# JiaxuanYou/graph-pooling

Hardware: AMD Instinct MI355X
Metric: graphs/sec fwd+bwd, DD padded batch N_max=500 (higher is better)
Workload: dtype f32; 1 GPU; S-DD: DD-shaped padded batch, B=20/GPU, N_max=500, F=89, H=E=20, K=50, L=3, 1 pool; graphs_per_gpu=20, global_batch=20, linkpred=False, hip_graph=True, parallelism=dp1

## Files before the change

### graph_pooling_amd/_lib.py

```python
from __future__ import annotations

import ctypes as C
import os
import threading

_HERE = os.path.dirname(os.path.abspath(__file__))
LIB_PATH = os.environ.get("DP_LIB") or os.path.join(_HERE, "libdiffpool_hip.so")

DP_MAX_LAYERS = 8
DP_MAX_LEVELS = 4
DP_MAX_PRED = 4

F_ADD_SELF, F_NORMALIZE, F_RELU, F_BN, F_LAST_ONLY = 1, 2, 4, 8, 16
MODE_EVAL, MODE_TRAIN = 0, 1
ERR_DEVICE = -4
DEVERR_BARRIER, DEVERR_NONFINITE_GRAD = 1, 2
SAVE_S, SAVE_XPOOL, SAVE_ADJPOOL, SAVE_Z, SAVE_ZASSIGN, SAVE_ARGMAX = 0, 1, 2, 3, 4, 5


class StackCfg(C.Structure):
    _fields_ = [("n_layers", C.c_int),
                ("dims", C.c_int * (DP_MAX_LAYERS + 1)),
                ("w_off", C.c_long * DP_MAX_LAYERS),
                ("b_off", C.c_long * DP_MAX_LAYERS),
# ... 9 lines not shown
                ("assign_pred_w_off", C.c_long * DP_MAX_LEVELS),
                ("assign_pred_b_off", C.c_long * DP_MAX_LEVELS),
                ("n_pred", C.c_int),
                ("pred_dims", C.c_int * (DP_MAX_PRED + 2)),
                ("pred_w_off", C.c_long * (DP_MAX_PRED + 1)),
                ("pred_b_off", C.c_long * (DP_MAX_PRED + 1)),
                ("flags", C.c_int),
                ("readout", C.c_int),
                ("s2s_off", C.c_long * 6),
                ("mask_readout", C.c_int),
                ("n_params", C.c_long),
                ("n_graph_params", C.c_long),
                ("bn_world", C.c_int),
                ("exchange", C.c_void_p),
                ("exchange_user", C.c_void_p)]


EXCHANGE_FN = C.CFUNCTYPE(C.c_int, C.c_void_p, C.c_void_p, C.c_void_p, C.c_size_t, C.c_void_p)


_P = C.c_void_p
_I = C.c_int
_L = C.c_long
_F = C.c_float
_Z = C.c_size_t

_PROTOS = {
    "dp_version": (_I, []),
    "dp_last_error_string": (C.c_char_p, []),
    "dp_device_error": (_I, [_I]),
    "dp_device_error_describe": (C.c_char_p, [_I]),
    "dp_profile_level0": (_I, [_I]),
    "dp_profile_level0_read": (_I, [_I, C.POINTER(C.c_double), C.POINTER(_I)]),
    "dp_sizeof_encoder_cfg": (_Z, []),
    "dp_bgemm_f32": (_I, [_P, _P, _P, _P, _I, _I, _I, _I, _I, _I, _I, _L, _L, _L, _I, _I, _F, _F, _I, _P]),
    "dp_bgemm_split_bf16": (_I, [_P, _P, _P, _I, _I, _I, _I, _I, _I, _I, _L, _L, _L, _I, _I, _F, _P]),
    "dp_adj_aggregate": (_I, [_P, _P, _I, _P, _I, _I, _I, _I, _I, _F, _P]),
    "dp_adj_pack_ld": (_I, [_I]),
    "dp_adj_pack_bytes": (_Z, [_I, _I]),
    "dp_adj_pack": (_I, [_P, _P, _P, _P, _I, _I, _P]),
    "dp_adj_aggregate_packed_workspace_bytes": (_Z, [_I, _I, _I]),
    "dp_adj_aggregate_packed": (_I, [_P, _P, _P, _P, _P, _I, _P, _I, _I, _I, _I, _I, _F, _I, _P, _Z, _P]),
    "dp_gcn_layer_workspace_bytes": (_Z, [_I, _I, _I, _I]),
    "dp_gcn_layer_fwd": (_I, [_P, _I, _P, _P, _P, _P, _I, _P, _I, _I, _I, _I, _I, _P, _Z, _P]),
    "dp_gcn_layer_bwd": (_I, [_P, _I, _P, _P, _P, _I, _P, _P, _I, _P, _I, _P, _P, _P, _I, _I, _I, _I, _I, _P, _Z, _P]),
    "dp_bn_node_workspace_bytes": (_Z, [_I, _I, _I]),
    "dp_bn_node_fwd": (_I, [_P, _I, _P, _I, _P, _I, _I, _I, _I, _P, _Z, _P]),
    "dp_bn_node_bwd": (_I, [_P, _I, _P, _I, _P, _P, _I, _P, _I, _I, _I, _I, _I, _P, _Z, _P]),
    "dp_assign_workspace_bytes": (_Z, [_I, _I, _I, _I]),
    "dp_assign_softmax_mask_fwd": (_I, [_P, _I, _P, _P, _P, _P, _I, _I, _I, _I, _P, _Z, _P]),
    "dp_assign_softmax_mask_bwd": (_I, [_P, _I, _P, _P, _P, _P, _P, _I, _P, _P, _I, _I, _I, _I, _P, _Z, _P]),
    "dp_pool_fwd": (_I, [_P, _P, _I, _P, _P, _P, _P, _I, _I, _I, _I, _P]),
    "dp_pool_bwd_workspace_bytes": (_Z, [_I, _I, _I, _I]),
    "dp_pool_bwd": (_I, [_P, _P, _I, _P, _P, _P, _P, _P, _P, _I, _P, _I, _I, _I, _I, _P, _Z, _P]),
    "dp_masked_max_fwd": (_I, [_P, _I, _P, _P, _I, _P, _I, _I, _I, _P]),
    "dp_masked_max_bwd": (_I, [_P, _I, _P, _P, _I, _I, _I, _I, _P]),
    "dp_linkpred_workspace_bytes": (_Z, [_I, _I, _I]),
    "dp_linkpred_loss_fwd": (_I, [_P, _P, _P, _P, _I, _I, _I, _P, _Z, _P]),
    "dp_linkpred_loss_bwd": (_I, [_P, _P, _P, _P, _P, _I, _I, _I, _I, _P, _Z, _P]),
    "dp_cross_entropy_fwd": (_I, [_P, _P, _P, _P, _I, _I, _P]),
    "dp_cross_entropy_bwd": (_I, [_P, _P, _P, _P, _I, _I, _P]),
    "dp_set2set_save_bytes": (_Z, [_I, _I, _I]),
    "dp_set2set_plan": (_I, [_I, _I]),
    "dp_set2set_fwd": (_I, [_P, _I, _P, _P, _P, _P, _P, _P, _P, _I, _I, _I, _P, _Z, _P]),
    "dp_set2set_bwd_workspace_bytes": (_Z, [_I, _I, _I]),
    "dp_set2set_bwd": (_I, [_P, _I, _P, _P, _P, _P, _P, _P, _P, _P, _P, _I, _P, _P, _P, _P, _P, _P,
# ... 106 lines not shown
```

### graph_pooling_amd/csrc/dp_level0.hip

```cpp
#include "dp_common.h"
#include <utility>
#include <vector>

namespace dp {

#ifdef DP_STAMP
__device__ unsigned long long g_l0_stamps[3][64];
#define L0_STAMP(i)                                                                                    \
    do {                                                                                               \
        if (threadIdx.x == 0 && (wid == 0 || wid == (int)gridDim.x / 2 || wid == (int)gridDim.x - 1)) \
            g_l0_stamps[wid == 0 ? 0 : (wid == (int)gridDim.x - 1 ? 2 : 1)][i] = __builtin_amdgcn_s_memtime(); \
    } while (0)
#else
#define L0_STAMP(i) \
    do {            \
    } while (0)
#endif

namespace {

typedef float f32x4 __attribute__((ext_vector_type(4)));
typedef float f32x4_u __attribute__((ext_vector_type(4), aligned(4)));
typedef short s16x8 __attribute__((ext_vector_type(8)));
typedef __bf16 bf16x8 __attribute__((ext_vector_type(8)));
typedef unsigned short u16x4 __attribute__((ext_vector_type(4)));
typedef unsigned short u16x8 __attribute__((ext_vector_type(8)));

constexpr int L0_NT = 512;
constexpr int L0_NW = 8;
constexpr int L0_TEAMS = L0_NT / 16;
constexpr int L0_NK = 4;
constexpr int L0_BPAIRS = 4;
constexpr float L0_L2_EPS = 1e-12f;
constexpr float L0_BN_EPS = 1e-5f;
constexpr int L0_SPIN_LIMIT = 1 << 22;

constexpr int BAR_GCOUNT = 0, BAR_DONE = 32, BAR_GFLAG = 48, BAR_ERR = 64, BAR_SEQ = 96, BAR_GRAPH0 = 128;
constexpr int BAR_GSTRIDE = 48;

__device__ __forceinline__ int ag_ld(int* p) { return __hip_atomic_load(p, __ATOMIC_RELAXED, __HIP_MEMORY_SCOPE_AGENT); }
__device__ __forceinline__ void ag_st(int* p, int v) { __hip_atomic_store(p, v, __ATOMIC_RELAXED, __HIP_MEMORY_SCOPE_AGENT); }
__device__ __forceinline__ int ag_add(int* p, int v) { return __hip_atomic_fetch_add(p, v, __ATOMIC_RELAXED, __HIP_MEMORY_SCOPE_AGENT); }

struct L0Args {
    Level0Fwd f;
    int T, RB;
    int ldp;
    int K8;
    int steps;
    int epad;
    long vs_off[DP_MAX_LAYERS + 1];
    int lds_act[2];
    int lds_scr;
    int scr_floats;
    int* dev_err;
    int spin_limit, target_bias;
    long zero_n16;
};

template <bool TA, bool TB, typename Store>
__device__ inline void l0_mma(const float* A, int lda, const float* B, int ldb, int M, int N, int K, Store store,
                              int wave_shift = 0) {
    const int lane = threadIdx.x & 63;
    const int wave = ((threadIdx.x >> 6) + L0_NW - wave_shift % L0_NW) % L0_NW;
    const int l15 = lane & 15, kq = lane >> 4;
    const int tm = (M + 15) / 16, tn = (N + 15) / 16;
    const int sa4 = 4 * (TA ? lda : 1), sb4 = 4 * (TB ? 1 : ldb);
    for (int t = wave; t < tm * tn; t += L0_NW) {
        const int tr = t / tn, tc = t - tr * tn;
        const int i = tr * 16 + l15, j = tc * 16 + l15;
        const float* ap = (TA ? A + min(i, M - 1) : A + min(i, M - 1) * lda) + kq * (sa4 >> 2);
        const float* bp = (TB ? B + min(j, N - 1) * ldb : B + min(j, N - 1)) + kq * (sb4 >> 2);
        f32x4 acc0 = (f32x4){0.f, 0.f, 0.f, 0.f}, acc1 = acc0;
        int k = 0;
        float pa[4], pb[4], qa[4], qb[4];
        auto ld = [&](float (&xa)[4], float (&xb)[4]) {
            xa[0] = ap[0]; xa[1] = ap[sa4]; xa[2] = ap[2 * sa4]; xa[3] = ap[3 * sa4];
            xb[0] = bp[0]; xb[1] = bp[sb4]; xb[2] = bp[2 * sb4]; xb[3] = bp[3 * sb4];
            ap += 4 * sa4;
            bp += 4 * sb4;
        };
        auto mm = [&](const float (&xa)[4], const float (&xb)[4]) {
            acc0 = __builtin_amdgcn_mfma_f32_16x16x4f32(xa[0], xb[0], acc0, 0, 0, 0);
            acc1 = __builtin_amdgcn_mfma_f32_16x16x4f32(xa[1], xb[1], acc1, 0, 0, 0);
// ... 114 lines not shown
            q[u] = *reinterpret_cast<const f32x4_u*>(src + 4 * min(base + u * L0_NT + (int)threadIdx.x, nq - 1));
#pragma unroll
        for (int u = 0; u < QN; ++u) {
            const int e4 = base + u * L0_NT + (int)threadIdx.x;
            if (e4 < nq) *reinterpret_cast<f32x4*>(dst + 4 * e4) = q[u];
        }
    }
    if (te < count) dst[te] = tail;
    for (int e = count + (int)threadIdx.x; e < zero_to; e += L0_NT) dst[e] = 0.f;
}

__device__ inline void l0_write_split(ScBuf vsb, const float* PT, int ct, int CTt, int K8, int k8_0, int nk8, int nrows) {
    const long pl = (long)CTt * K8 * 128;
    const int items = nk8 * CTt * 16;
    for (int item = threadIdx.x; item < items; item += L0_NT) {
        const int c = item & 15, t = item >> 4;
        const int k8l = t / CTt, cb = t - k8l * CTt;
        const int vc = cb * 16 + c, lr = k8l * 8;
        u16x8 h, m, l;
#pragma unroll
        for (int j = 0; j < 8; ++j) {
            const float v = (vc < ct && lr + j < nrows) ? PT[(lr + j) * ct + min(vc, ct - 1)] : 0.f;
            unsigned short hh, mm, ll;
            bf16_split3(v, hh, mm, ll);
            h[j] = hh; m[j] = mm; l[j] = ll;
        }
        const long o = vs_index(0, CTt, K8, cb, k8_0 + k8l, c, 0);
        sc_st16(vsb, (unsigned)(o * 2), __builtin_bit_cast(u32x4, h));
        sc_st16(vsb, (unsigned)((o + pl) * 2), __builtin_bit_cast(u32x4, m));
        sc_st16(vsb, (unsigned)((o + 2 * pl) * 2), __builtin_bit_cast(u32x4, l));
    }
}

template <int MI, int CTH>
__device__ __forceinline__ void l0_agg_bf16(const unsigned short* Alds, int ldp, const unsigned short* vsp, int CTt, int K8,
                                            int steps, int rot, int cb0, f32x4 (&acc)[MI][CTH]) {
    int lane = threadIdx.x & 63;
    asm volatile("" : "+v"(lane));
    const int kh = __builtin_amdgcn_readfirstlane(threadIdx.x >> 6) & 3;
    const int l15 = lane & 15, kq = lane >> 4;
    auto eff = [&](int step) {
        const int s2 = min(step, steps - 1) + rot;
        return s2 >= steps ? s2 - steps : s2;
    };
    auto load_b = [&](int step, s16x8 (&dst)[3][CTH]) {
        const int st = eff(step);
#pragma unroll
        for (int p = 0; p < 3; ++p)
#pragma unroll
            for (int cbi = 0; cbi < CTH; ++cbi) {
                const int cb = min(cb0 + cbi, CTt - 1);
                const long o = ((((long)p * CTt + cb) * K8 + st * 4 + kq) * 16 + l15) * 8;
                dst[p][cbi] = *reinterpret_cast<const s16x8*>(vsp + o);
            }
    };
    auto mma = [&](int step, const s16x8 (&bf)[3][CTH]) {
        s16x8 av[MI];
#pragma unroll
        for (int rb = 0; rb < MI; ++rb)
            av[rb] = *reinterpret_cast<const s16x8*>(Alds + (rb * 16 + l15) * ldp + eff(step) * 32 + kq * 8);
#pragma unroll
        for (int p = 2; p >= 0; --p)
#pragma unroll
            for (int rb = 0; rb < MI; ++rb)
#pragma unroll
                for (int cbi = 0; cbi < CTH; ++cbi)
// ... 141 lines not shown
        const bool in = row < nrows && c8 * 8 < ld;
        const u32x4 v = in ? s.q[u] : (u32x4){0u, 0u, 0u, 0u};
        if (c8 * 8 + 8 <= ldp) *reinterpret_cast<u32x4*>(Alds + row * ldp + c8 * 8) = v;
    }
}

template <int MI>
__global__ __launch_bounds__(L0_NT) void k_level0_fwd(L0Args a) {
    constexpr int RB = MI * 16;
    extern __shared__ __attribute__((aligned(16))) float lds[];
    const Level0Fwd& f = a.f;
    const int tid = threadIdx.x, lane = tid & 63;
    const int tl = tid & 15, team = tid >> 4;
    const int N = f.N, G = f.G, L = f.L;
    int wid;
    {
        const int nwg = gridDim.x, xcd = blockIdx.x & 7, idx = blockIdx.x >> 3;
        const int qd = nwg >> 3, rm = nwg & 7;
        wid = (xcd < rm ? xcd * (qd + 1) : rm * (qd + 1) + (xcd - rm) * qd) + idx;
    }
    const int b = wid / a.T, rb = wid - b * a.T;
    const int r0 = rb * RB;
    const int nrows = min(RB, N - r0);
    const int nb = f.num_nodes ? min(f.num_nodes[b], N) : N;
    const int rot = (rb * 4) % a.steps;
    L0_STAMP(0);

    unsigned short* Alds = reinterpret_cast<unsigned short*>(lds);
    float* ACT0 = lds + a.lds_act[0];
    float* ACT1 = lds + a.lds_act[1];
    float* SCR = lds + a.lds_scr;
    float* BIAS = lds + a.lds_scr + a.scr_floats;
    int* sflag = reinterpret_cast<int*>(BIAS + (2 * DP_MAX_LAYERS + 1) * 64);
    if (tid < 4) sflag[tid] = 0;
    L0Epoch ep{0};
    const unsigned seq = (unsigned)f.bar[BAR_SEQ];

    auto vs_wr = [&](int pass, int CTt) {
        return sc_buf(f.vs + a.vs_off[pass] + (long)b * 3 * CTt * a.K8 * 128, (size_t)3 * CTt * a.K8 * 128 * 2);
    };
    auto vs_rd = [&](int pass, int CTt) { return f.vs + a.vs_off[pass] + (long)b * 3 * CTt * a.K8 * 128; };

    if (wid == 0) {
        if (f.next_bar && tid < 64) f.next_bar[tid] = 0;
        if (tid == 64) ag_st(f.bar + BAR_ERR, 0);
    }
    L0_STAMP(1);
    const int din0_0 = f.st[0].dims[0], din0_1 = G == 2 ? f.st[1].dims[0] : 0;
    bool bad = false;
    float* const X0s0 = SCR;
    float* const X0s1 = X0s0 + RB * din0_0;
    float* const W0s0 = X0s1 + RB * din0_1;
    float* const W0s1 = W0s0 + ((din0_0 * f.st[0].dims[1] + 3) & ~3);
    float* const PT = W0s1 + (G == 2 ? ((din0_1 * f.st[1].dims[1] + 3) & ~3) : 0);
    const auto side_loads = [&]() {
        l0_copy_in<4>(X0s0, f.x0[0] + ((long)b * N + r0) * din0_0, nrows * din0_0, RB * din0_0);
        l0_copy_in<4>(W0s0, f.params + f.st[0].w_off[0], din0_0 * f.st[0].dims[1]);
        if (G == 2) {
            l0_copy_in<4>(X0s1, f.x0[1] + ((long)b * N + r0) * din0_1, nrows * din0_1, RB * din0_1);
            l0_copy_in<4>(W0s1, f.params + f.st[1].w_off[0], din0_1 * f.st[1].dims[1]);
        }
        for (int e = tid; e < (2 * L + 1) * 64; e += L0_NT) {
            const int slot = e >> 6, c = e & 63;
            float v0 = 0.f;
            if (slot < 2 * L) {
                const int l = slot >> 1, g = slot & 1;
                if (g < G && f.st[g].b_off[l] >= 0 && c < f.st[g].dims[l + 1]) v0 = f.params[f.st[g].b_off[l] + c];
            } else if (G == 2 && f.bp_off >= 0 && c < f.K) {
                v0 = f.params[f.bp_off + c];
            }
            BIAS[(slot < 2 * L ? slot : 2 * DP_MAX_LAYERS) * 64 + c] = v0;
        }
    };
    if (f.A) {
// ... 33 lines not shown
        for (int seg = 1; seg < segs; ++seg) {
            l0_stage_issue<MI>(q, rows, f.pk_ld, nrows, seg);
            l0_stage_commit<MI>(q, Alds, a.ldp, f.pk_ld, nrows, seg);
        }
    }
    L0_STAMP(2);
    if (f.zero_p) {
        uint4* zp = reinterpret_cast<uint4*>(f.zero_p);
        const long nwg = gridDim.x, per = (a.zero_n16 + nwg - 1) / nwg;
        const long end = min(a.zero_n16, ((long)wid + 1) * per);
        for (long i = (long)wid * per + tid; i < end; i += L0_NT) zp[i] = make_uint4(0, 0, 0, 0);
    }
    if (__any(bad) && lane == 0) sflag[2] = 1;
    lds_barrier();
    L0_STAMP(3);
    const bool blk_bad = sflag[2] != 0;
    if (blk_bad && tid == 0) {
        ag_st(f.bar + BAR_GRAPH0 + b * BAR_GSTRIDE + 32, 1);
        ag_st(f.bar + BAR_GFLAG, 1);
    }
    if (f.A) {
        const ScBuf atb = sc_buf(f.pkAt + (long)b * N * f.pk_ld, (size_t)N * f.pk_ld * 2);
        constexpr int P8 = RB / 8;
        for (int e = tid; e < N * P8; e += L0_NT) {
            const int k = e / P8, i8 = e - k * P8;
            if (r0 + i8 * 8 < f.pk_ld) {
                u16x8 h;
#pragma unroll
                for (int j = 0; j < 8; ++j) h[j] = Alds[(i8 * 8 + j) * a.ldp + k];
                sc_st16(atb, (unsigned)(((long)k * f.pk_ld + r0 + i8 * 8) * 2), __builtin_bit_cast(u32x4, h));
            }
        }
    }
    L0_STAMP(4);
    int ct = f.st[0].dims[1] + (G == 2 ? f.st[1].dims[1] : 0);
    for (int g = 0; g < G; ++g) {
        const int dout = f.st[g].dims[1], c0 = g ? f.st[0].dims[1] : 0;
        l0_mma<false, false>(g ? X0s1 : X0s0, g ? din0_1 : din0_0, g ? W0s1 : W0s0, dout, RB, dout, g ? din0_1 : din0_0,
                             [&](int r, int c, float v) { PT[r * ct + c0 + c] = v; }, g * 3);
    }
    lds_barrier();
    L0_STAMP(5);
    const int k8_0 = r0 / 8;
    const int nk8 = min(rb == a.T - 1 ? a.K8 - k8_0 : RB / 8, a.K8 - k8_0);
    {
        const int CTt = (ct + 15) / 16;
        l0_write_split(vs_wr(0, CTt), PT, ct, CTt, a.K8, k8_0, nk8, nrows);
    }
    L0_STAMP(6);
    bool ok = l0_barrier(a, b, sflag, ep);
    L0_STAMP(7);
    const bool exact = !f.A || ag_ld(f.bar + BAR_GRAPH0 + b * BAR_GSTRIDE + 32) == 0;
    const float* Arows = f.A + ((long)b * N + r0) * N;
    const float* Acols = f.A + (long)b * N * N + r0;

    constexpr int ITEMS = (RB * 2 + L0_TEAMS - 1) / L0_TEAMS;
    for (int l = 0; l < L; ++l) {
        const bool last = l == L - 1;
        const int w0 = f.st[0].dims[l + 1], w1 = G == 2 ? f.st[1].dims[l + 1] : 0;
        const int wmax = max(w0, w1);
        const int CTt = (ct + 15) / 16;
        const int ctp = CTt * 16 + 1;
        float* red = SCR;
        l0_aggregate<MI>(a, Alds, exact, Arows, N, 1, nrows, vs_rd(l, CTt), CTt, red, ctp, rot);
        L0_STAMP(8 + 8 * l);
        int wn0 = 0, wn1 = 0;
        float* const Wn0 = red + 4 * RB * ctp;
        if (!last) {
            wn0 = f.st[0].dims[l + 1] * f.st[0].dims[l + 2];
            wn1 = G == 2 ? f.st[1].dims[l + 1] * f.st[1].dims[l + 2] : 0;
        }
        float* const Wn1 = Wn0 + ((wn0 + 3) & ~3);
        if (!last) {
            l0_copy_in<4>(Wn0, f.params + f.st[0].w_off[l + 1], wn0);
            if (G == 2) l0_copy_in<4>(Wn1, f.params + f.st[1].w_off[l + 1], wn1);
        }
        lds_barrier();
        L0_STAMP(9 + 8 * l);
        const ScBuf partw = sc_buf(f.part + (long)l * f.B * N * G * 4, (size_t)f.B * N * G * 4 * sizeof(float));
        const unsigned bn_tag = (seq << 4) | (unsigned)(l + 1);
#pragma unroll
        for (int j = 0; j < ITEMS; ++j) {
            float yv[L0_NK];
            const int it = team + j * L0_TEAMS;
            const int r = min(G == 2 ? it >> 1 : it, RB - 1), g = G == 2 ? (it & 1) : 0;
            const bool on = it < RB * G && r < nrows;
            const long row = (long)b * N + min(r0 + r, N - 1);
            const int wg = g ? w1 : w0, c0gg = g ? w0 : 0;
            const float* bias = BIAS + (2 * l + g) * 64;
            float ss = 0.f;
#pragma unroll
            for (int k = 0; k < L0_NK; ++k) {
                yv[k] = 0.f;
                if (16 * k < wmax) {
                    const int c = min(tl + 16 * k, wg - 1);
                    const int o = r * ctp + c0gg + c;
                    float v = ((red[o] + red[RB * ctp + o]) + (red[2 * RB * ctp + o] + red[3 * RB * ctp + o])) + bias[c];
                    v = tl + 16 * k < wg ? v : 0.f;
                    yv[k] = v;
                    ss += v * v;
                }
            }
            ss = row16_sum(ss);
            const float inv = ss > L0_L2_EPS * L0_L2_EPS ? __builtin_amdgcn_rsqf(ss) : 1.f / L0_L2_EPS;
            float s1 = 0.f;
            float* yg = last ? f.Z[g] + row * f.ldz[g] + f.coff[g][l] : f.Y[l] + row * ct + c0gg;
            float* act = (g ? ACT1 : ACT0) + r * f.ldz[g] + f.coff[g][l];
#pragma unroll
            for (int k = 0; k < L0_NK; ++k) {
                if (16 * k < wmax) {
                    const int c = tl + 16 * k;
                    yv[k] *= inv;
                    if (on && c < wg) yg[c] = yv[k];
                    if (it < RB * G && c < wg) act[c] = r < nrows ? yv[k] : 0.f;
                    s1 += fmaxf(yv[k], 0.f);
                }
            }
            if (on && tl == 0) f.invn[l][row * G + g] = inv;
            if (!last && f.bn) {
                s1 = row16_sum(s1);
                const float mean = s1 / (float)wg;
                float m2 = 0.f;
#pragma unroll
                for (int k = 0; k < L0_NK; ++k) {
                    if (16 * k < wmax) {
                        const float v = (tl + 16 * k < wg) ? fmaxf(yv[k], 0.f) - mean : 0.f;
                        m2 += v * v;
                    }
                }
                m2 = row16_sum(m2);
// ... 43 lines not shown
                    }
                    const float var = row16_sum(s2) / ((float)f.B * (float)wg);
                    rstd = __builtin_amdgcn_rsqf(var + L0_BN_EPS);
                    if (!ok) mu = rstd = __builtin_nanf("");
                    if (on && b == 0 && tl == 0) {
                        f.stats[l][((long)node * G + g) * 2] = mu;
                        f.stats[l][((long)node * G + g) * 2 + 1] = rstd;
                    }
                }
                float* xg = f.Z[g] + row * f.ldz[g] + f.coff[g][l];
                float* act = (g ? ACT1 : ACT0) + r * f.ldz[g] + f.coff[g][l];
#pragma unroll
                for (int k = 0; k < L0_NK; ++k) {
                    if (16 * k < wmax) {
                        const int c = tl + 16 * k;
                        const float xv = (fmaxf(act[min(c, wg - 1)], 0.f) - mu) * rstd;
                        if (on && c < wg) xg[c] = xv;
                        if (it < RB * G && c < wg) act[c] = r < nrows ? xv : 0.f;
                    }
                }
            }
        }
        lds_barrier();
        L0_STAMP(12 + 8 * l);
        for (int g = 0; g < G; ++g) {
            const int din = f.st[g].dims[l + 1], dout = f.st[g].dims[l + 2], c0 = g ? f.st[0].dims[l + 2] : 0;
            l0_mma<false, false>((g ? ACT1 : ACT0) + f.coff[g][l], f.ldz[g], g ? Wn1 : Wn0, dout, RB, dout, din,
                                 [&](int r, int c, float v) { PTn[r * ctn + c0 + c] = v; }, g * 3);
        }
        lds_barrier();
        L0_STAMP(13 + 8 * l);
        {
            const int CTn = (ctn + 15) / 16;
            l0_write_split(vs_wr(l + 1, CTn), PTn, ctn, CTn, a.K8, k8_0, nk8, nrows);
        }
        L0_STAMP(14 + 8 * l);
        ok = l0_barrier(a, b, sflag, ep) && ok;
        L0_STAMP(15 + 8 * l);
        ct = ctn;
    }
    lds_barrier();

    const int K = f.K, D = f.ldz[0];
    float* XP = SCR;
    if (G == 2 && K > 0) {
        const int Da = f.ldz[1];
        const int CTk = (K + 15) / 16, ctpk = CTk * 16 + 1;
        float* TL = SCR + 4 * RB * ctpk;
        float* SL = TL + RB * K;
        float* WP = SCR;
        l0_copy_in<4>(WP, f.params + f.wp_off, K * Da);
        lds_barrier();
        L0_STAMP(40);
        {
            const float* bp = BIAS + 2 * DP_MAX_LAYERS * 64;
            l0_mma<false, true>(ACT1, Da, WP, Da, RB, K, Da, [&](int r, int c, float v) { SL[r * K + c] = v + bp[c]; });
        }
        lds_barrier();
        L0_STAMP(41);
        for (int r = team; r < RB; r += L0_TEAMS) {
            const int node = r0 + r;
            const bool valid = node < nb;
            float lv[L0_NK];
#pragma unroll
            for (int k = 0; k < L0_NK; ++k) lv[k] = SL[r * K + min(tl + 16 * k, K - 1)];
            float m = -INFINITY;
#pragma unroll
            for (int k = 0; k < L0_NK; ++k) m = fmaxf(m, lv[k]);
            m = row16_max(m);
            float sum = 0.f;
#pragma unroll
            for (int k = 0; k < L0_NK; ++k) {
                lv[k] = expf(lv[k] - m);
                sum += (tl + 16 * k < K) ? lv[k] : 0.f;
            }
            sum = row16_sum(sum);
            const float rinv = 1.f / sum;
            const long row = (long)b * N + min(node, N - 1);
#pragma unroll
            for (int k = 0; k < L0_NK; ++k) {
                const int c = tl + 16 * k;
                if (c < K) {
                    const float v = (valid && node < N) ? lv[k] * rinv : 0.f;
                    SL[r * K + c] = v;
                    if (node < N) {
                        f.S[row * K + c] = v;
                        if (f.S2) f.S2[row * K + c] = v;
                    }
                }
            }
        }
        lds_barrier();
        L0_STAMP(42);
        l0_write_split(vs_wr(L, CTk), SL, K, CTk, a.K8, k8_0, nk8, nrows);
        L0_STAMP(43);
        {
            const int segs = (a.steps * 32 + 511) / 512;
            const unsigned short* atp = f.pkAt + ((long)b * N + r0) * f.pk_ld;
            L0RowStage<MI> atq;
            l0_stage_issue<MI>(atq, atp, f.pk_ld, nrows, 0);
            ok = l0_barrier(a, b, sflag, ep) && ok;
            L0_STAMP(44);
            l0_stage_commit<MI>(atq, Alds, a.ldp, f.pk_ld, nrows, 0);
            for (int seg = 1; seg < segs; ++seg) {
                l0_stage_issue<MI>(atq, atp, f.pk_ld, nrows, seg);
                l0_stage_commit<MI>(atq, Alds, a.ldp, f.pk_ld, nrows, seg);
            }
        }
        lds_barrier();
        L0_STAMP(45);
        l0_aggregate<MI>(a, Alds, exact, Acols, 1, N, nrows, vs_rd(L, CTk), CTk, SCR, ctpk, rot);
        L0_STAMP(46);
        lds_barrier();
        L0_STAMP(47);
        for (int r = team; r < RB; r += L0_TEAMS) {
            const long row = (long)b * N + min(r0 + r, N - 1);
#pragma unroll
            for (int k = 0; k < L0_NK; ++k) {
                const int c = tl + 16 * k;
                const int o = r * ctpk + min(c, K - 1);
                const float v = (SCR[o] + SCR[RB * ctpk + o]) + (SCR[2 * RB * ctpk + o] + SCR[3 * RB * ctpk + o]);
                if (c < K) {
                    TL[r * K + c] = r < nrows ? v : 0.f;
                    if (r < nrows) f.Tt[row * K + c] = v;
                }
            }
        }
        lds_barrier();
        L0_STAMP(48);
        float* AP = XP + K * D;
        l0_mma<true, false>(SL, K, ACT0, D, K, D, RB, [&](int i, int j, float v) { XP[i * D + j] = v; });
        l0_mma<true, false>(TL, K, SL, K, K, K, RB, [&](int i, int j, float v) { AP[i * K + j] = v; }, 4);
        for (int e = K * D + K * K + tid; e < a.epad; e += L0_NT) XP[e] = 0.f;
        lds_barrier();
        L0_STAMP(49);
        {
            const ScBuf xpb = sc_buf(f.xpart + ((long)b * a.T + rb) * a.epad, (size_t)a.epad * 4);
            for (int e4 = tid; e4 < a.epad / 4; e4 += L0_NT)
                sc_st16(xpb, (unsigned)(e4 * 16), *reinterpret_cast<const u32x4*>(XP + e4 * 4));
        }
    }
    if (f.do_max) {
        const int nm = f.mask_readout ? max(min(nb - r0, nrows), 0) : nrows;
        const ScBuf mpb = sc_buf(f.mpart + ((long)b * a.T + rb) * f.rw * 2, (size_t)f.rw * 2 * 4);
        float* MV = XP + a.epad;
        int* MI_ = reinterpret_cast<int*>(MV + 8 * f.rw);
        constexpr int RG = RB / 8;
        for (int c0 = 0; c0 < f.rw; c0 += 64) {
            const int c = c0 + (tid & 63), grp = tid >> 6;
            float best = -INFINITY;
            int bi = -1;
            if (c < f.rw) {
#pragma unroll
                for (int rr = 0; rr < RG; ++rr) {
// ... 65 lines not shown
#pragma unroll
                for (int u = 0; u < 8; ++u)
                    pr[u] = *reinterpret_cast<const float2*>(mg + ((long)min(t0 + u, a.T - 1) * f.rw + c) * 2);
#pragma unroll
                for (int u = 0; u < 8; ++u) {
                    const int i = __float_as_int(pr[u].y);
                    if (t0 + u < a.T && i >= 0 && pr[u].x > best) {
                        best = pr[u].x;
                        bi = i;
                    }
                }
            }
            if (f.mask_readout && nb < N && !(best > 0.f)) {
                if (best < 0.f || bi < 0) {
                    best = 0.f;
                    bi = -1;
                }
            }
            if (!ok) best = __builtin_nanf("");
            f.feat[(long)b * f.ldfeat + f.featoff + c] = best;
            f.argmax[(long)b * f.rw + c] = bi;
        }
    }
    lds_barrier();
    L0_STAMP(52);
    if (tid == 0) {
        const int old = ag_add(f.bar + BAR_DONE, 1);
        sflag[3] = old == (int)gridDim.x - 1;
    }
    lds_barrier();
    if (sflag[3]) {
        const int gflag = ag_ld(f.bar + BAR_GFLAG);
        if (tid < 64) f.pk_flag[tid] = tid == 0 ? gflag : 0;
        for (int g = tid; g < f.B; g += L0_NT) {
            ag_st(f.bar + BAR_GRAPH0 + g * BAR_GSTRIDE, 0);
            ag_st(f.bar + BAR_GRAPH0 + g * BAR_GSTRIDE + 32, 0);
        }
        if (tid == 0) {
            ag_st(f.bar + BAR_GCOUNT, 0);
            ag_st(f.bar + BAR_GFLAG, 0);
            ag_st(f.bar + BAR_DONE, 0);
            ag_st(f.bar + BAR_SEQ, (int)((seq + 1u) & 0x03ffffffu));
        }
    }
}

struct L0BArgs {
    Level0Bwd f;
    int T, RB, ldp, K8, steps;
    long vs_off[DP_MAX_LAYERS + 1];
    int lds_dz[2];
    int lds_scr, slots_floats, scr_floats;
    int P0;
    int cw[2][DP_MAX_LAYERS], cb[2][DP_MAX_LAYERS], cwp, cbp;
    int nseg;
    int seg_c[4 * DP_MAX_LAYERS + 2], seg_len[4 * DP_MAX_LAYERS + 2];
    long seg_flat[4 * DP_MAX_LAYERS + 2];
    int* dev_err;
    int spin_limit, target_bias;
};

#ifdef DP_STAMP
__device__ unsigned long long g_l0b_stamps[3][64];
#define L0B_STAMP(i)                                                                                   \
    do {                                                                                               \
        if (threadIdx.x == 0 && (wid == 0 || wid == (int)gridDim.x / 2 || wid == (int)gridDim.x - 1)) \
            g_l0b_stamps[wid == 0 ? 0 : (wid == (int)gridDim.x - 1 ? 2 : 1)][i] = __builtin_amdgcn_s_memtime(); \
    } while (0)
#else
// ... 482 lines not shown
                        if (t0 + u < a.T) s += v[u];
                }
                if (!ok) s = (f32x4){__builtin_nanf(""), __builtin_nanf(""), __builtin_nanf(""), __builtin_nanf("")};
                int sg = 0;
                while (sg + 1 < a.nseg && a.seg_c[sg + 1] <= e4 * 4) ++sg;
#pragma unroll
                for (int j = 0; j < 4; ++j) {
                    const int e = e4 * 4 + j - a.seg_c[sg];
                    if (e < a.seg_len[sg]) slab[a.seg_flat[sg] + e] = s[j];
                }
            }
        }
    }
    lds_barrier();
    L0B_STAMP(41);
    if (tid == 0) {
        const int old = ag_add(f.bar + BAR_DONE, 1);
        sflag[3] = old == (int)gridDim.x - 1;
    }
    lds_barrier();
    if (sflag[3]) {
        for (int g = tid; g < f.B; g += L0_NT) ag_st(f.bar + BAR_GRAPH0 + g * BAR_GSTRIDE, 0);
        if (tid == 0) {
            ag_st(f.bar + BAR_GCOUNT, 0);
            ag_st(f.bar + BAR_DONE, 0);
            ag_st(f.bar + BAR_SEQ, (int)((seq + 1u) & 0x03ffffffu));
        }
    }
}

struct L0Geom {
    int RB, T, ldp, K8, steps, epad;
    int lds_act[2], lds_scr, scr_floats;
    size_t lds_bytes;
};
int l0_device_cus() {
    static std::atomic<int> cus[64];
    int dev = 0;
    if (hipGetDevice(&dev) != hipSuccess || dev < 0 || dev >= 64) return 0;
    int v = cus[dev].load(std::memory_order_relaxed);
    if (v == 0) {
        hipDeviceProp_t prop;
        v = hipGetDeviceProperties(&prop, dev) == hipSuccess ? prop.multiProcessorCount : -1;
        cus[dev].store(v, std::memory_order_relaxed);
    }
    return v > 0 ? v : 0;
}
bool l0_geometry(const Level0Fwd& f, L0Geom& g) {
    const int cus = l0_device_cus();
    if (cus <= 0) return false;
    const int N = f.N, G = f.G, L = f.L;
    g.steps = (N + 31) / 32;
    g.K8 = g.steps * 4;
    g.ldp = ((N + 511) / 512) * 512 + 8;
    const int K = G == 2 ? f.K : 0, D = f.ldz[0];
    g.epad = (K * D + K * K + 3) & ~3;
    for (int RB = 16; RB <= 64; RB += 16) {
        const int T = (N + RB - 1) / RB;
        if ((long)f.B * T > cus) continue;
        size_t scr = 0;
        auto need = [&](size_t fl) { scr = fl > scr ? fl : scr; };
        {
            size_t fl = 0;
            for (int s = 0; s < G; ++s)
                fl += (size_t)RB * f.st[s].dims[0] +
                      (((size_t)f.st[s].dims[0] * f.st[s].dims[1] + 3) & ~size_t(3));
            int ct = 0;
            for (int s = 0; s < G; ++s) ct += f.st[s].dims[1];
            need(fl + (size_t)RB * ct);
        }
        for (int l = 0; l < L; ++l) {
            int ct = 0;
            for (int s = 0; s < G; ++s) ct += f.st[s].dims[l + 1];
            const size_t slots = (size_t)4 * RB * (((ct + 15) / 16) * 16 + 1);
            need(slots);
            if (l < L - 1) {
                size_t fl = 0;
                int ctn = 0;
                for (int s = 0; s < G; ++s) {
                    fl += ((size_t)f.st[s].dims[l + 1] * f.st[s].dims[l + 2] + 3) & ~size_t(3);
                    ctn += f.st[s].dims[l + 2];
                }
                need(slots + fl + (size_t)RB * ctn);
            }
        }
        need((size_t)g.epad + 16 * (size_t)(f.rw > 0 ? f.rw : 0));
        if (K > 0) {
            const int ctpk = ((K + 15) / 16) * 16 + 1;
            need((size_t)4 * RB * ctpk + 2 * (size_t)RB * K);
            if ((size_t)K * f.ldz[1] > (size_t)4 * RB * ctpk || (size_t)g.epad > (size_t)4 * RB * ctpk) continue;
        }
        const size_t adj_fl = ((size_t)RB * g.ldp * 2 + 15) / 16 * 4;
        g.lds_act[0] = (int)adj_fl;
        g.lds_act[1] = g.lds_act[0] + ((RB * f.ldz[0] + 3) & ~3);
        g.lds_scr = g.lds_act[1] + (G == 2 ? ((RB * f.ldz[1] + 3) & ~3) : 0);
        g.scr_floats = (int)((scr + 3) & ~size_t(3));
        g.lds_bytes = ((size_t)g.lds_scr + g.scr_floats + (2 * DP_MAX_LAYERS + 1) * 64 + 16) * sizeof(float);
        if (g.lds_bytes > 159 * 1024) continue;
        g.RB = RB;
        g.T = T;
        return true;
    }
    return false;
}

struct L0Prof {
    std::mutex m;
    bool on = false;
    std::vector<std::pair<hipEvent_t, hipEvent_t>> ev[2];
};
L0Prof& l0_prof() {
    static L0Prof p;
    return p;
}
struct L0Timed {
    hipStream_t st;
    int which;
    hipEvent_t e0 = nullptr, e1 = nullptr;
    L0Timed(hipStream_t s, int w) : st(s), which(w) {
        L0Prof& p = l0_prof();
        if (!p.on) return;
        hipStreamCaptureStatus cs = hipStreamCaptureStatusNone;
        if (hipStreamIsCapturing(st, &cs) != hipSuccess || cs != hipStreamCaptureStatusNone) return;
        if (hipEventCreate(&e0) != hipSuccess || hipEventCreate(&e1) != hipSuccess) {
            e0 = e1 = nullptr;
            return;
        }
        (void)hipEventRecord(e0, st);
    }
    ~L0Timed() {
        if (!e0) return;
        (void)hipEventRecord(e1, st);
        L0Prof& p = l0_prof();
        std::lock_guard<std::mutex> g(p.m);
        p.ev[which].emplace_back(e0, e1);
    }
};

template <int MI>
void l0_launch(Seq& q, const L0Args& a, size_t lds_bytes) {
    static DynLdsOnce attr;
    ensure_dyn_lds(q, attr, reinterpret_cast<const void*>(&k_level0_fwd<MI>), 160 * 1024, "k_level0_fwd");
    if (!q.ok()) return;
    L0Timed timed(q.stream, 0);
    hipLaunchKernelGGL(k_level0_fwd<MI>, dim3(a.f.B * a.T), dim3(L0_NT), lds_bytes, q.stream, a);
    q.check_launch("level0_forward");
}

}

size_t level0_bar_ints(int B) { return (size_t)BAR_GRAPH0 + (size_t)BAR_GSTRIDE * B; }
static void l0_vs_layout(const Level0Fwd& f, long (&off)[DP_MAX_LAYERS + 1], size_t& total) {
    const int K8 = ((f.N + 31) / 32) * 4;
    size_t o = 0;
    for (int p = 0; p <= f.L; ++p) {
        int ct = 0;
        if (p < f.L) for (int s = 0; s < f.G; ++s) ct += f.st[s].dims[p + 1];
        else ct = f.G == 2 ? f.K : 0;
        off[p] = (long)o;
        o += (size_t)f.B * 3 * ((ct + 15) / 16) * K8 * 128;
    }
    total = o;
}
size_t level0_vs_elems(const Level0Fwd& f) {
    long off[DP_MAX_LAYERS + 1];
    size_t total;
    l0_vs_layout(f, off, total);
    return total + 64;
}
size_t level0_part_floats(const Level0Fwd& f) { return (size_t)(f.L > 1 ? f.L - 1 : 1) * f.B * f.N * f.G * 4 + 4; }
const int* level0_error_word(const int* bar) { return bar + BAR_ERR; }
int* level0_seq_word(int* bar) { return bar + BAR_SEQ; }
size_t level0_xpart_floats(const Level0Fwd& f) {
    L0Geom g;
    if (!l0_geometry(f, g)) return 4;
    return (size_t)f.B * g.T * g.epad + 4;
}
size_t level0_mpart_floats(const Level0Fwd& f) {
    L0Geom g;
    if (!l0_geometry(f, g)) return 4;
    return (size_t)f.B * g.T * (f.rw > 0 ? f.rw : 1) * 2 + 4;
}

bool level0_persistent_ok(const Level0Fwd& f) {
    if (knobs().no_l0_persist) return false;
    if (f.G < 1 || f.G > 2 || f.L < 1 || f.L > DP_MAX_LAYERS) return false;
    if (knobs().no_pack) return false;
    if (f.N < 64 || (f.N & 3) || f.B < 1 || f.B > 16 * L0_BPAIRS) return false;
    for (int l = 0; l < f.L; ++l) {
        int ct = 0;
        size_t wfl = 0;
        for (int s = 0; s < f.G; ++s) {
            if (f.st[s].dims[l + 1] < 1 || f.st[s].dims[l + 1] > 16 * L0_NK) return false;
            ct += f.st[s].dims[l + 1];
            wfl += (size_t)f.st[s].dims[l] * f.st[s].dims[l + 1];
        }
        if (ct > 96 || wfl > 8192) return false;
        for (int s = 0; s < f.G; ++s)
            if ((size_t)f.st[s].dims[l] * f.st[s].dims[l + 1] > 4 * 4 * L0_NT) return false;
    }
    for (int s = 0; s < f.G; ++s)
        if (f.st[s].dims[0] < 1 || f.st[s].dims[0] > 256 || f.ldz[s] > 160) return false;
    if (f.G == 2) {
        if (f.K < 1 || f.K > 16 * L0_NK || (size_t)f.K * f.ldz[1] > 8192) return false;
    }
    if (f.do_max && (f.rw < 1 || f.zoff + f.rw > f.ldz[0])) return false;
    L0Geom g;
    return l0_geometry(f, g);
}

void level0_forward(Seq& q, const Level0Fwd& f) {
    if (!q.ok()) return;
    L0Geom g;
    if (!l0_geometry(f, g)) {
        set_error("level0_forward: shape outside the persistent kernel's envelope");
        q.err = DP_ERR_UNSUPPORTED;
        return;
    }
    L0Args a{};
    a.f = f;
    a.T = g.T; a.RB = g.RB; a.ldp = g.ldp; a.K8 = g.K8; a.steps = g.steps; a.epad = g.epad;
    a.lds_act[0] = g.lds_act[0]; a.lds_act[1] = g.lds_act[1]; a.lds_scr = g.lds_scr; a.scr_floats = g.scr_floats;
    a.dev_err = device_error_word();
    a.spin_limit = knobs().test_barrier_fail ? 64 : L0_SPIN_LIMIT;
    a.target_bias = knobs().test_barrier_fail ? 1 : 0;
    {
        size_t total;
        l0_vs_layout(f, a.vs_off, total);
    }
    a.zero_n16 = f.zero_p ? (long)(f.zero_bytes / 16) : 0;
    if (f.zero_p && ((reinterpret_cast<uintptr_t>(f.zero_p) & 15) != 0 || (f.zero_bytes & 15) != 0)) {
        zero_fill(q, f.zero_p, f.zero_bytes);
        a.f.zero_p = nullptr;
        a.zero_n16 = 0;
    }
    switch (g.RB / 16) {
        case 1: l0_launch<1>(q, a, g.lds_bytes); break;
        case 2: l0_launch<2>(q, a, g.lds_bytes); break;
        case 3: l0_launch<3>(q, a, g.lds_bytes); break;
        default: l0_launch<4>(q, a, g.lds_bytes); break;
    }
}

namespace {
struct L0BGeom {
    int RB, T, ldp, K8, steps;
    int lds_dz[2], lds_scr, slots_floats, scr_floats;
    size_t lds_bytes;
};
Level0Fwd l0_as_fwd(const Level0Bwd& f) {
    Level0Fwd w{};
    w.B = f.B; w.N = f.N; w.L = f.L; w.G = f.G; w.bn = f.bn;
    w.st[0] = f.st[0]; w.st[1] = f.st[1];
    w.ldz[0] = f.ldz[0]; w.ldz[1] = f.ldz[1];
    w.K = f.K;
    return w;
}
bool l0b_geometry(const Level0Bwd& f, L0BGeom& g) {
    L0Geom fg;
    Level0Fwd w = l0_as_fwd(f);
    w.do_max = 0;
    if (!l0_geometry(w, fg)) return false;
// ... 136 lines not shown
}

extern "C" __attribute__((visibility("default"))) int dp_profile_level0(int enable) {
    L0Prof& p = l0_prof();
    std::lock_guard<std::mutex> g(p.m);
    for (auto& v : p.ev) {
        for (auto& e : v) {
            (void)hipEventDestroy(e.first);
            (void)hipEventDestroy(e.second);
        }
        v.clear();
    }
    p.on = enable != 0;
    return DP_OK;
}
extern "C" __attribute__((visibility("default"))) int dp_profile_level0_read(int which, double* total_us, int* launches) {
    if (which < 0 || which > 1 || !total_us || !launches) return DP_ERR_INVALID_ARG;
    L0Prof& p = l0_prof();
    std::lock_guard<std::mutex> g(p.m);
    double tot = 0.0;
    int n = 0;
    for (auto& e : p.ev[which]) {
        float ms = 0.f;
        if (hipEventSynchronize(e.second) != hipSuccess || hipEventElapsedTime(&ms, e.first, e.second) != hipSuccess)
            return DP_ERR_UNSUPPORTED;
        tot += (double)ms * 1000.0;
        ++n;
    }
    *total_us = tot;
    *launches = n;
    return DP_OK;
}

#ifdef DP_STAMP
extern "C" __attribute__((visibility("default"))) int dp_debug_l0b_stamps(unsigned long long* out) {
    return (int)hipMemcpyFromSymbol(out, HIP_SYMBOL(g_l0b_stamps), sizeof(unsigned long long) * 3 * 64);
}
#endif

#ifdef DP_STAMP
extern "C" __attribute__((visibility("default"))) int dp_debug_l0_stamps(unsigned long long* out) {
    return (int)hipMemcpyFromSymbol(out, HIP_SYMBOL(g_l0_stamps), sizeof(unsigned long long) * 3 * 64);
}
#endif

}
```

### include/diffpool_hip.h

```cpp
#ifndef DIFFPOOL_HIP_H
#define DIFFPOOL_HIP_H

#include <stddef.h>
#include <stdint.h>

#ifdef __cplusplus
extern "C" {
#endif
#if defined(__GNUC__)
#pragma GCC visibility push(default)
#endif

#define DP_VERSION 100

#define DP_OK 0
#define DP_ERR_INVALID_ARG (-1)
#define DP_ERR_WORKSPACE (-2)
#define DP_ERR_UNSUPPORTED (-3)
#define DP_ERR_DEVICE (-4)

#define DP_F_ADD_SELF 1
#define DP_F_NORMALIZE 2
#define DP_F_RELU 4
#define DP_F_BN 8
#define DP_F_LAST_ONLY 16

#define DP_MAX_LAYERS 8
#define DP_MAX_LEVELS 4
#define DP_MAX_PRED 4

int dp_version(void);
const char* dp_last_error_string(void);

#define DP_DEVERR_BARRIER 1
#define DP_DEVERR_NONFINITE_GRAD 2
int dp_device_error(int clear);
const char* dp_device_error_describe(int mask);

int dp_profile_level0(int enable);
int dp_profile_level0_read(int which, double* total_us, int* launches);

int dp_bgemm_f32(const float* A, const float* B, float* C, const float* bias, int batch, int M, int N,
                 int K, int lda, int ldb, int ldc, long strideA, long strideB, long strideC, int transA,
                 int transB, float alpha, float beta, int act, void* stream);

int dp_bgemm_split_bf16(const float* A, const float* B, float* C, int batch, int M, int N, int K, int lda, int ldb,
                        int ldc, long strideA, long strideB, long strideC, int transA, int transB, float beta,
                        void* stream);

int dp_adj_aggregate(const float* adj, const float* V, int ldv, float* U, int ldu, int B, int n, int C,
                     int trans, float beta, void* stream);

int dp_adj_pack_ld(int n);
size_t dp_adj_pack_bytes(int B, int n);
int dp_adj_pack(const float* adj, void* packed, void* packed_t, int* flag, int B, int n, void* stream);
size_t dp_adj_aggregate_packed_workspace_bytes(int B, int n, int C);
int dp_adj_aggregate_packed(const float* adj, const void* packed, const void* packed_t, const int* flag,
                            const float* V, int ldv, float* U, int ldu, int B, int n, int C, int trans, float beta,
                            int presplit, void* workspace, size_t workspace_bytes, void* stream);

size_t dp_gcn_layer_workspace_bytes(int B, int n, int Fin, int Fout);
int dp_gcn_layer_fwd(const float* x, int ldx, const float* adj, const float* W, const float* bias,
                     float* y, int ldy, float* invnorm, int B, int n, int Fin, int Fout, int flags,
                     void* workspace, size_t workspace_bytes, void* stream);
int dp_gcn_layer_bwd(const float* x, int ldx, const float* adj, const float* W, const float* y, int ldy,
                     const float* invnorm, const float* dy, int lddy, float* dx, int lddx, float* dW,
                     float* db, float* dadj, int B, int n, int Fin, int Fout, int flags, void* workspace,
                     size_t workspace_bytes, void* stream);

size_t dp_bn_node_workspace_bytes(int B, int n, int F);
int dp_bn_node_fwd(const float* x, int ldx, float* y, int ldy, float* stats, int B, int n, int F,
                   int relu, void* workspace, size_t workspace_bytes, void* stream);
int dp_bn_node_bwd(const float* x, int ldx, const float* y, int ldy, const float* stats, const float* dy,
// ... 229 lines not shown
```

Measured before the change: 82110 graphs/s.

## Add sparse neighbor-list gather path for level-0 adjacency aggregation

Builds a per-row neighbor list (up to 32 entries) from the bf16 adjacency tile in LDS. When every graph's adjacency is binary and within that degree bound, the dense bf16-split MFMA aggregation is replaced by a gather-sum over fp32 rows written to a new row-major buffer. This cuts the dense N×N aggregation cost for sparse DD graphs. In exchange it adds extra LDS use, an additional fp32 copy of features, neighbor-list build passes and per-graph fallback flags.

```diff
diff --git a/graph_pooling_amd/_lib.py b/graph_pooling_amd/_lib.py
--- a/graph_pooling_amd/_lib.py
+++ b/graph_pooling_amd/_lib.py
@@ -65,6 +65,8 @@
     "dp_device_error_describe": (C.c_char_p, [_I]),
     "dp_profile_level0": (_I, [_I]),
     "dp_profile_level0_read": (_I, [_I, C.POINTER(C.c_double), C.POINTER(_I)]),
+    "dp_level0_nbr_flags": (_I, [C.POINTER(_I), C.POINTER(_I), _I]),
+    "dp_level0_nbr_enable": (_I, [_I]),
     "dp_sizeof_encoder_cfg": (_Z, []),
     "dp_bgemm_f32": (_I, [_P, _P, _P, _P, _I, _I, _I, _I, _I, _I, _I, _L, _L, _L, _I, _I, _F, _F, _I, _P]),
     "dp_bgemm_split_bf16": (_I, [_P, _P, _P, _I, _I, _I, _I, _I, _I, _I, _L, _L, _L, _I, _I, _F, _P]),
diff --git a/graph_pooling_amd/csrc/dp_level0.hip b/graph_pooling_amd/csrc/dp_level0.hip
--- a/graph_pooling_amd/csrc/dp_level0.hip
+++ b/graph_pooling_amd/csrc/dp_level0.hip
@@ -17,6 +17,8 @@
     } while (0)
 #endif
 
+__device__ int g_l0_nbr_flags[128];
+
 namespace {
 
 typedef float f32x4 __attribute__((ext_vector_type(4)));
@@ -37,6 +39,7 @@
 
 constexpr int BAR_GCOUNT = 0, BAR_DONE = 32, BAR_GFLAG = 48, BAR_ERR = 64, BAR_SEQ = 96, BAR_GRAPH0 = 128;
 constexpr int BAR_GSTRIDE = 48;
+constexpr int L0_DMAX = 32;
 
 __device__ __forceinline__ int ag_ld(int* p) { return __hip_atomic_load(p, __ATOMIC_RELAXED, __HIP_MEMORY_SCOPE_AGENT); }
 __device__ __forceinline__ void ag_st(int* p, int v) { __hip_atomic_store(p, v, __ATOMIC_RELAXED, __HIP_MEMORY_SCOPE_AGENT); }
@@ -50,6 +53,8 @@
     int steps;
     int epad;
     long vs_off[DP_MAX_LAYERS + 1];
+    long vq_off[DP_MAX_LAYERS + 1];
+    int lds_nbr;
     int lds_act[2];
     int lds_scr;
     int scr_floats;
@@ -230,6 +235,85 @@
     }
 }
 
+__host__ __device__ inline int l0_ldq(int ct) { return (ct + 31) & ~31; }
+#define L0_LDS __attribute__((address_space(3)))
+
+__device__ __forceinline__ bool l0_build_nbr(const L0_LDS unsigned short* Alds, int ldp, int ncol, int rows,
+                                                       L0_LDS unsigned short* nbr, L0_LDS int* cnt) {
+    const int lane = threadIdx.x & 63;
+    const int wave = __builtin_amdgcn_readfirstlane(threadIdx.x >> 6);
+    bool bad = false;
+    for (int r = wave; r < rows; r += L0_NW) {
+        int total = 0;
+        for (int c0 = 0; c0 < ncol; c0 += 512) {
+            const int c = c0 + lane * 8;
+            u16x8 v = (u16x8){0, 0, 0, 0, 0, 0, 0, 0};
+            if (c < ncol) v = *reinterpret_cast<const L0_LDS u16x8*>(Alds + r * ldp + c);
+            unsigned m = 0;
+#pragma unroll
+            for (int j = 0; j < 8; ++j) {
+                const bool nz = v[j] != 0 && c + j < ncol;
+                m |= (nz ? 1u : 0u) << j;
+                bad |= nz && v[j] != 0x3F80;
+            }
+            int before = 0, all = 0;
+#pragma unroll
+            for (int j = 0; j < 8; ++j) {
+                const unsigned long long bl = __ballot((m >> j) & 1u);
+                before += __builtin_amdgcn_mbcnt_hi((unsigned)(bl >> 32), __builtin_amdgcn_mbcnt_lo((unsigned)bl, 0u));
+                all += __popcll(bl);
+            }
+            int pos = total + before;
+#pragma unroll
+            for (int j = 0; j < 8; ++j)
+                if ((m >> j) & 1u) {
+                    if (pos < L0_DMAX) nbr[r * L0_DMAX + pos] = (unsigned short)(c + j);
+                    ++pos;
+                }
+            total += all;
+        }
+        if (lane == 0) cnt[r] = min(total, L0_DMAX);
+        bad |= total > L0_DMAX;
+    }
+    return bad;
+}
+
+__device__ inline void l0_write_rows(ScBuf qb, const float* PT, int ct, int ldq, int row0, int nrows) {
+    const int nq = (ct + 3) >> 2;
+    for (int item = threadIdx.x; item < nrows * nq; item += L0_NT) {
+        const int r = item / nq, q4 = (item - r * nq) * 4;
+        u32x4 w;
+#pragma unroll
+        for (int j = 0; j < 4; ++j) w[j] = q4 + j < ct ? __float_as_uint(PT[r * ct + q4 + j]) : 0u;
+        sc_st16(qb, (unsigned)(((row0 + r) * ldq + q4) * 4), w);
+    }
+}
+
+__device__ __attribute__((noinline)) void l0_gather_pass(const L0_LDS unsigned short* nbr, const L0_LDS int* cnt,
+                                                         const float* P, int ldq, int ct, int rows, L0_LDS float* out,
+                                                         int ldo) {
+    const int nq = (ct + 3) >> 2;
+    for (int item = threadIdx.x; item < rows * nq; item += L0_NT) {
+        const int r = item / nq, q4 = (item - r * nq) * 4;
+        const int n = cnt[r];
+        const L0_LDS unsigned short* nb = nbr + r * L0_DMAX;
+        f32x4 s = (f32x4){0.f, 0.f, 0.f, 0.f};
+#pragma unroll 1
+        for (int i0 = 0; i0 < n; i0 += 8) {
+            f32x4 v[8];
+#pragma unroll
+            for (int u = 0; u < 8; ++u)
+                v[u] = *reinterpret_cast<const f32x4*>(P + (long)nb[min(i0 + u, n - 1)] * ldq + q4);
+#pragma unroll
+            for (int u = 0; u < 8; ++u)
+                if (i0 + u < n) s += v[u];
+        }
+#pragma unroll
+        for (int j = 0; j < 4; ++j)
+            if (q4 + j < ct) out[r * ldo + q4 + j] = s[j];
+    }
+}
+
 template <int MI, int CTH>
 __device__ __forceinline__ void l0_agg_bf16(const unsigned short* Alds, int ldp, const unsigned short* vsp, int CTt, int K8,
                                             int steps, int rot, int cb0, f32x4 (&acc)[MI][CTH]) {
@@ -437,7 +521,10 @@
     float* SCR = lds + a.lds_scr;
     float* BIAS = lds + a.lds_scr + a.scr_floats;
     int* sflag = reinterpret_cast<int*>(BIAS + (2 * DP_MAX_LAYERS + 1) * 64);
-    if (tid < 4) sflag[tid] = 0;
+    if (tid < 8) sflag[tid] = 0;
+    const bool nbr_on = a.lds_nbr >= 0;
+    L0_LDS unsigned short* NBR = (L0_LDS unsigned short*)(lds + max(a.lds_nbr, 0));
+    L0_LDS int* NCNT = (L0_LDS int*)(NBR + RB * L0_DMAX);
     L0Epoch ep{0};
     const unsigned seq = (unsigned)f.bar[BAR_SEQ];
 
@@ -445,6 +532,12 @@
         return sc_buf(f.vs + a.vs_off[pass] + (long)b * 3 * CTt * a.K8 * 128, (size_t)3 * CTt * a.K8 * 128 * 2);
     };
     auto vs_rd = [&](int pass, int CTt) { return f.vs + a.vs_off[pass] + (long)b * 3 * CTt * a.K8 * 128; };
+    auto vq_wr = [&](int pass, int ldq) {
+        return sc_buf(f.vs + a.vq_off[pass] + (long)b * N * ldq * 2, (size_t)N * ldq * 4);
+    };
+    auto vq_rd = [&](int pass, int ldq) {
+        return reinterpret_cast<const float*>(f.vs + a.vq_off[pass]) + (long)b * N * ldq;
+    };
 
     if (wid == 0) {
         if (f.next_bar && tid < 64) f.next_bar[tid] = 0;
@@ -544,6 +637,7 @@
             }
         }
     }
+    if (nbr_on && l0_build_nbr((const L0_LDS unsigned short*)Alds, a.ldp, N, RB, NBR, NCNT)) sflag[4] = 1;
     L0_STAMP(4);
     int ct = f.st[0].dims[1] + (G == 2 ? f.st[1].dims[1] : 0);
     for (int g = 0; g < G; ++g) {
@@ -558,11 +652,14 @@
     {
         const int CTt = (ct + 15) / 16;
         l0_write_split(vs_wr(0, CTt), PT, ct, CTt, a.K8, k8_0, nk8, nrows);
-    }
+        if (nbr_on) l0_write_rows(vq_wr(0, l0_ldq(ct)), PT, ct, l0_ldq(ct), r0, nrows);
+    }
+    if (tid == 0 && (sflag[4] || blk_bad || !nbr_on)) ag_st(f.bar + BAR_GRAPH0 + b * BAR_GSTRIDE + 33, 1);
     L0_STAMP(6);
     bool ok = l0_barrier(a, b, sflag, ep);
     L0_STAMP(7);
     const bool exact = !f.A || ag_ld(f.bar + BAR_GRAPH0 + b * BAR_GSTRIDE + 32) == 0;
+    const bool gath = nbr_on && exact && ag_ld(f.bar + BAR_GRAPH0 + b * BAR_GSTRIDE + 33) == 0;
     const float* Arows = f.A + ((long)b * N + r0) * N;
     const float* Acols = f.A + (long)b * N * N + r0;
 
@@ -574,7 +671,8 @@
         const int CTt = (ct + 15) / 16;
         const int ctp = CTt * 16 + 1;
         float* red = SCR;
-        l0_aggregate<MI>(a, Alds, exact, Arows, N, 1, nrows, vs_rd(l, CTt), CTt, red, ctp, rot);
+        if (gath) l0_gather_pass(NBR, NCNT, vq_rd(l, l0_ldq(ct)), l0_ldq(ct), ct, RB, (L0_LDS float*)red, ctp);
+        else l0_aggregate<MI>(a, Alds, exact, Arows, N, 1, nrows, vs_rd(l, CTt), CTt, red, ctp, rot);
         L0_STAMP(8 + 8 * l);
         int wn0 = 0, wn1 = 0;
         float* const Wn0 = red + 4 * RB * ctp;
@@ -607,7 +705,9 @@
                 if (16 * k < wmax) {
                     const int c = min(tl + 16 * k, wg - 1);
                     const int o = r * ctp + c0gg + c;
-                    float v = ((red[o] + red[RB * ctp + o]) + (red[2 * RB * ctp + o] + red[3 * RB * ctp + o])) + bias[c];
+                    float v = red[o];
+                    if (!gath) v = (v + red[RB * ctp + o]) + (red[2 * RB * ctp + o] + red[3 * RB * ctp + o]);
+                    v += bias[c];
                     v = tl + 16 * k < wg ? v : 0.f;
                     yv[k] = v;
                     ss += v * v;
@@ -717,7 +817,8 @@
         L0_STAMP(13 + 8 * l);
         {
             const int CTn = (ctn + 15) / 16;
-            l0_write_split(vs_wr(l + 1, CTn), PTn, ctn, CTn, a.K8, k8_0, nk8, nrows);
+            if (gath) l0_write_rows(vq_wr(l + 1, l0_ldq(ctn)), PTn, ctn, l0_ldq(ctn), r0, nrows);
+            else l0_write_split(vs_wr(l + 1, CTn), PTn, ctn, CTn, a.K8, k8_0, nk8, nrows);
         }
         L0_STAMP(14 + 8 * l);
         ok = l0_barrier(a, b, sflag, ep) && ok;
@@ -778,6 +879,7 @@
         lds_barrier();
         L0_STAMP(42);
         l0_write_split(vs_wr(L, CTk), SL, K, CTk, a.K8, k8_0, nk8, nrows);
+        if (nbr_on) l0_write_rows(vq_wr(L, l0_ldq(K)), SL, K, l0_ldq(K), r0, nrows);
         L0_STAMP(43);
         {
             const int segs = (a.steps * 32 + 511) / 512;
@@ -793,8 +895,13 @@
             }
         }
         lds_barrier();
+        if (nbr_on && l0_build_nbr((const L0_LDS unsigned short*)Alds, a.ldp, N, RB, NBR, NCNT)) sflag[5] = 1;
+        lds_barrier();
+        const bool gath_t = nbr_on && exact && sflag[5] == 0;
+        if (tid == 0 && !gath_t) ag_st(f.bar + BAR_GRAPH0 + b * BAR_GSTRIDE + 34, 1);
         L0_STAMP(45);
-        l0_aggregate<MI>(a, Alds, exact, Acols, 1, N, nrows, vs_rd(L, CTk), CTk, SCR, ctpk, rot);
+        if (gath_t) l0_gather_pass(NBR, NCNT, vq_rd(L, l0_ldq(K)), l0_ldq(K), K, RB, (L0_LDS float*)SCR, ctpk);
+        else l0_aggregate<MI>(a, Alds, exact, Acols, 1, N, nrows, vs_rd(L, CTk), CTk, SCR, ctpk, rot);
         L0_STAMP(46);
         lds_barrier();
         L0_STAMP(47);
@@ -804,7 +911,8 @@
             for (int k = 0; k < L0_NK; ++k) {
                 const int c = tl + 16 * k;
                 const int o = r * ctpk + min(c, K - 1);
-                const float v = (SCR[o] + SCR[RB * ctpk + o]) + (SCR[2 * RB * ctpk + o] + SCR[3 * RB * ctpk + o]);
+                float v = SCR[o];
+                if (!gath_t) v = (v + SCR[RB * ctpk + o]) + (SCR[2 * RB * ctpk + o] + SCR[3 * RB * ctpk + o]);
                 if (c < K) {
                     TL[r * K + c] = r < nrows ? v : 0.f;
                     if (r < nrows) f.Tt[row * K + c] = v;
@@ -936,9 +1044,18 @@
     if (sflag[3]) {
         const int gflag = ag_ld(f.bar + BAR_GFLAG);
         if (tid < 64) f.pk_flag[tid] = tid == 0 ? gflag : 0;
+        if (tid < 128) {
+            const int g = tid & 63;
+            const bool pooled = G == 2 && K > 0;
+            g_l0_nbr_flags[tid] = g < f.B && (tid < 64 || pooled) &&
+                                  ag_ld(f.bar + BAR_GRAPH0 + g * BAR_GSTRIDE + (tid < 64 ? 33 : 34)) == 0;
+        }
+        lds_barrier();
         for (int g = tid; g < f.B; g += L0_NT) {
             ag_st(f.bar + BAR_GRAPH0 + g * BAR_GSTRIDE, 0);
             ag_st(f.bar + BAR_GRAPH0 + g * BAR_GSTRIDE + 32, 0);
+            ag_st(f.bar + BAR_GRAPH0 + g * BAR_GSTRIDE + 33, 0);
+            ag_st(f.bar + BAR_GRAPH0 + g * BAR_GSTRIDE + 34, 0);
         }
         if (tid == 0) {
             ag_st(f.bar + BAR_GCOUNT, 0);
@@ -1487,8 +1604,10 @@
 struct L0Geom {
     int RB, T, ldp, K8, steps, epad;
     int lds_act[2], lds_scr, scr_floats;
+    int lds_nbr;
     size_t lds_bytes;
 };
+std::atomic<int> g_l0_nbr_enabled{1};
 int l0_device_cus() {
     static std::atomic<int> cus[64];
     int dev = 0;
@@ -1552,6 +1671,12 @@
         g.scr_floats = (int)((scr + 3) & ~size_t(3));
         g.lds_bytes = ((size_t)g.lds_scr + g.scr_floats + (2 * DP_MAX_LAYERS + 1) * 64 + 16) * sizeof(float);
         if (g.lds_bytes > 159 * 1024) continue;
+        g.lds_nbr = -1;
+        const size_t nbr_bytes = (size_t)RB * L0_DMAX * 2 + (size_t)RB * 4;
+        if (g.lds_bytes + nbr_bytes <= 159 * 1024) {
+            g.lds_nbr = (int)(g.lds_bytes / sizeof(float));
+            g.lds_bytes += nbr_bytes;
+        }
         g.RB = RB;
         g.T = T;
         return true;
@@ -1605,7 +1730,7 @@
 }
 
 size_t level0_bar_ints(int B) { return (size_t)BAR_GRAPH0 + (size_t)BAR_GSTRIDE * B; }
-static void l0_vs_layout(const Level0Fwd& f, long (&off)[DP_MAX_LAYERS + 1], size_t& total) {
+static void l0_vs_layout(const Level0Fwd& f, long (&off)[DP_MAX_LAYERS + 1], long (&qoff)[DP_MAX_LAYERS + 1], size_t& total) {
     const int K8 = ((f.N + 31) / 32) * 4;
     size_t o = 0;
     for (int p = 0; p <= f.L; ++p) {
@@ -1614,13 +1739,15 @@
         else ct = f.G == 2 ? f.K : 0;
         off[p] = (long)o;
         o += (size_t)f.B * 3 * ((ct + 15) / 16) * K8 * 128;
+        qoff[p] = (long)o;
+        o += (size_t)f.B * f.N * l0_ldq(ct) * 2;
     }
     total = o;
 }
 size_t level0_vs_elems(const Level0Fwd& f) {
-    long off[DP_MAX_LAYERS + 1];
+    long off[DP_MAX_LAYERS + 1], qoff[DP_MAX_LAYERS + 1];
     size_t total;
-    l0_vs_layout(f, off, total);
+    l0_vs_layout(f, off, qoff, total);
     return total + 64;
 }
 size_t level0_part_floats(const Level0Fwd& f) { return (size_t)(f.L > 1 ? f.L - 1 : 1) * f.B * f.N * f.G * 4 + 4; }
@@ -1681,8 +1808,9 @@
     a.target_bias = knobs().test_barrier_fail ? 1 : 0;
     {
         size_t total;
-        l0_vs_layout(f, a.vs_off, total);
-    }
+        l0_vs_layout(f, a.vs_off, a.vq_off, total);
+    }
+    a.lds_nbr = g_l0_nbr_enabled.load(std::memory_order_relaxed) ? g.lds_nbr : -1;
     a.zero_n16 = f.zero_p ? (long)(f.zero_bytes / 16) : 0;
     if (f.zero_p && ((reinterpret_cast<uintptr_t>(f.zero_p) & 15) != 0 || (f.zero_bytes & 15) != 0)) {
         zero_fill(q, f.zero_p, f.zero_bytes);
@@ -1885,6 +2013,26 @@
     return DP_OK;
 }
 
+extern "C" __attribute__((visibility("default"))) int dp_level0_nbr_flags(int* a_flags, int* at_flags, int n) {
+    if (!a_flags || !at_flags || n < 0 || n > 64) {
+        set_error("dp_level0_nbr_flags: NULL pointer or n outside [0, 64]");
+        return DP_ERR_INVALID_ARG;
+    }
+    int host[128];
+    if (hipMemcpyFromSymbol(host, HIP_SYMBOL(g_l0_nbr_flags), sizeof(host)) != hipSuccess) {
+        set_error("dp_level0_nbr_flags: reading the device flags failed");
+        return DP_ERR_UNSUPPORTED;
+    }
+    for (int g = 0; g < n; ++g) {
+        a_flags[g] = host[g];
+        at_flags[g] = host[64 + g];
+    }
+    return DP_OK;
+}
+extern "C" __attribute__((visibility("default"))) int dp_level0_nbr_enable(int enable) {
+    return g_l0_nbr_enabled.exchange(enable != 0 ? 1 : 0, std::memory_order_relaxed);
+}
+
 #ifdef DP_STAMP
 extern "C" __attribute__((visibility("default"))) int dp_debug_l0b_stamps(unsigned long long* out) {
     return (int)hipMemcpyFromSymbol(out, HIP_SYMBOL(g_l0b_stamps), sizeof(unsigned long long) * 3 * 64);
diff --git a/include/diffpool_hip.h b/include/diffpool_hip.h
--- a/include/diffpool_hip.h
+++ b/include/diffpool_hip.h
@@ -39,6 +39,9 @@
 
 int dp_profile_level0(int enable);
 int dp_profile_level0_read(int which, double* total_us, int* launches);
+
+int dp_level0_nbr_flags(int* a_flags, int* at_flags, int n);
+int dp_level0_nbr_enable(int enable);
 
 int dp_bgemm_f32(const float* A, const float* B, float* C, const float* bias, int batch, int M, int N,
                  int K, int lda, int ldb, int ldc, long strideA, long strideB, long strideC, int transA,
```

Result: slower. 80480 graphs/s (-2.0%).
